# Ledicia/Molecular-Dynamics-Simulation---Lennard-Jones-monoatomic-fluid

Hardware: AMD Instinct MI355X
Metric: md_steps_per_sec_n262144_fp64 (higher is better)
Workload: dtype f64

## Files before the change

### molecular-dynamics-simulation---lennard-jones-monoatomic-fluid_amd/csrc/ljmd_kernels.hip

```cpp
#include <hip/hip_runtime.h>
#include <stdint.h>

#include "ljmd_internal.h"

namespace ljmdk {

__device__ __forceinline__ double wave_min(double v)
{
#pragma unroll
    for (int off = 32; off > 0; off >>= 1) v = fmin(v, __shfl_down(v, off, 64));
    return v;
}

__device__ __forceinline__ double wave_max(double v)
{
#pragma unroll
    for (int off = 32; off > 0; off >>= 1) v = fmax(v, __shfl_down(v, off, 64));
    return v;
}

__global__ __launch_bounds__(kBlock) void pair_rows_generic_kernel(PairArgs a)
{
    __shared__ double red[2 * kWavesPerBlock];
    const int row = blockIdx.x * kBlock + threadIdx.x;
    const double *own = a.pos + (size_t)a.rank * 3 * a.P;
    const double xi = own[row], yi = own[a.P + row], zi = own[2 * (size_t)a.P + row];

    double ax = 0.0, ay = 0.0, az = 0.0, s12 = 0.0, s6 = 0.0;

    const int j0 = blockIdx.y * a.chunk;
    const int j1 = min(j0 + a.chunk, a.n);
    for (int j = j0; j < j1;) {
        const int g = j / a.S;
        const int jl = j - g * a.S;
        const int jend = min(j1, (g + 1) * a.S);
        const double *bx = a.pos + (size_t)g * 3 * a.P;
        const double *by = bx + a.P, *bz = by + a.P;
        const int cnt = jend - j;
        const bool own_block = (g == a.rank);
        for (int k = 0; k < cnt; ++k) {
            const double dx0 = xi - bx[jl + k], dy0 = yi - by[jl + k], dz0 = zi - bz[jl + k];
            const double dx = dx0 - a.L * __builtin_round(dx0 * a.invL);
            const double dy = dy0 - a.L * __builtin_round(dy0 * a.invL);
            const double dz = dz0 - a.L * __builtin_round(dz0 * a.invL);
            const double r2 = dx * dx + dy * dy + dz * dz;
            if (r2 < a.rc2 && !(own_block && jl + k == row)) {
                const double u = 1.0 / r2;
                const double u3 = u * u * u;
                const double u6 = u3 * u3;
                s12 += u6;
                s6 += u3;
                const double mdu = 2.0 * u6 - u3;
                ax += mdu * dx * u;
                ay += mdu * dy * u;
                az += mdu * dz * u;
            }
        }
        j = jend;
    }

    double *s = a.slab + (size_t)blockIdx.y * 3 * a.P;
    s[row] = ax;
    s[a.P + row] = ay;
    s[2 * (size_t)a.P + row] = az;
    double v[2] = {s12, s6};
    block_sum<2>(v, red);
    if (threadIdx.x == 0) {
        double *w = a.wg_part + 2 * ((size_t)blockIdx.y * gridDim.x + blockIdx.x);
        w[0] = v[0];
        w[1] = v[1];
    }
}

__device__ __forceinline__ double axis_gap(double lo, double hi, double L)
{
    double g = __builtin_inf();
#pragma unroll
    for (int m = -2; m <= 2; ++m) {
        const double c = m * L;
        if (lo <= c && c <= hi) return 0.0;
        g = fmin(g, fmin(fabs(lo - c), fabs(hi - c)));
    }
    return g;
}

__device__ __forceinline__ double tile_gap2(const double *bbox, int I, int J, double L)
{
    const double *bi = bbox + (size_t)I * kBoxStride;
    const double *bj = bbox + (size_t)J * kBoxStride;
    double d2 = 0.0;
#pragma unroll
    for (int k = 0; k < 3; ++k) {
        const double g = axis_gap(bi[k] - bj[3 + k], bi[3 + k] - bj[k], L);
        d2 += g * g;
    }
    return d2;
}

__global__ __launch_bounds__(kBlock) void pair_tiles_kernel(PairArgs a)
{
    __shared__ double red[2 * kWavesPerBlock];
    const int lane = threadIdx.x & 63;
    const int wave = __builtin_amdgcn_readfirstlane(threadIdx.x >> 6);
    const int Il = blockIdx.x * kWavesPerBlock + wave;
    const int I = a.rank * a.TB + Il;
    const int row = Il * kTile + lane;
    const double *own = a.pos + (size_t)a.rank * 3 * a.P;
    const double xi = own[row], yi = own[a.P + row], zi = own[2 * (size_t)a.P + row];

    double ax = 0.0, ay = 0.0, az = 0.0, s12 = 0.0, s6 = 0.0;

    const uint64_t *mrow = a.mask + (size_t)Il * a.W;
    const int J0 = blockIdx.y * a.chunk, J1 = min(J0 + a.chunk, a.T);
    for (int w = J0 >> 6; w <= (J1 - 1) >> 6 && J0 < J1; ++w) {
        uint64_t m;
        if (a.inline_mask) {
            const int Jl = w * 64 + lane;
            const bool keep = Jl < a.T && (!(tile_gap2(a.bbox, I, Jl, a.L) > a.rc2_skin) || Jl == I);
            m = __ballot(keep);
        } else {
            m = mrow[w];
        }
        const int lo = max(J0 - w * 64, 0), hi = min(J1 - w * 64, 64);
        m &= (hi >= 64 ? ~0ull : ((1ull << hi) - 1ull)) & ~((1ull << lo) - 1ull);
        while (m) {
            const int b = __builtin_ctzll(m);
            m &= m - 1;
            const int J = w * 64 + b;
            const int gj = (a.G == 1) ? 0 : J / a.TB;
            const int jl = (J - gj * a.TB) * kTile;
            const double *bx = a.pos + (size_t)gj * 3 * a.P + jl;
            const double *by = bx + a.P, *bz = by + a.P;
            if (J == I) {
                for (int j0 = 0; j0 < kTile; j0 += 8) {
                    double xj[8], yj[8], zj[8];
#pragma unroll
                    for (int k = 0; k < 8; ++k) { xj[k] = bx[j0 + k]; yj[k] = by[j0 + k]; zj[k] = bz[j0 + k]; }
#pragma unroll
                    for (int k = 0; k < 8; ++k)
                        pair_fast<true>(xi, yi, zi, xj[k], yj[k], zj[k], a.L, a.invL, a.rc2, j0 + k == lane,
                                        ax, ay, az, s12, s6);
                }
            } else {
                for (int j0 = 0; j0 < kTile; j0 += 8) {
                    double xj[8], yj[8], zj[8];
#pragma unroll
                    for (int k = 0; k < 8; ++k) { xj[k] = bx[j0 + k]; yj[k] = by[j0 + k]; zj[k] = bz[j0 + k]; }
#pragma unroll
                    for (int k = 0; k < 8; ++k)
                        pair_fast<false>(xi, yi, zi, xj[k], yj[k], zj[k], a.L, a.invL, a.rc2, false,
                                         ax, ay, az, s12, s6);
                }
            }
        }
    }

    double *s = a.slab + (size_t)blockIdx.y * 3 * a.P;
    s[row] = ax;
    s[a.P + row] = ay;
    s[2 * (size_t)a.P + row] = az;
    double v[2] = {s12, s6};
    block_sum<2>(v, red);
    if (threadIdx.x == 0) {
        double *w = a.wg_part + 2 * ((size_t)blockIdx.y * gridDim.x + blockIdx.x);
        w[0] = v[0];
        w[1] = v[1];
    }
}


__device__ __forceinline__ double dpp_rotate(double v)
{
    int lo = __double2loint(v), hi = __double2hiint(v);
    lo = __builtin_amdgcn_update_dpp(lo, lo, 0x13C , 0xF, 0xF, false);
    hi = __builtin_amdgcn_update_dpp(hi, hi, 0x13C, 0xF, 0xF, false);
    return __hiloint2double(hi, lo);
}

__device__ __forceinline__ double straddle(double e, double half)
{
    return e - __builtin_copysign(half, e);
}

template <int NU>
__device__ __forceinline__ void pair_disp(double xi, double yi, double zi, double xj, double yj, double zj, double L,
                                          double invL, double sx, double sy, double sz, double &dx, double &dy, double &dz)
{
    static_assert(NU == 7 || NU == 8 || NU == 32 || NU == 33 || NU == 34 || NU == 40, "pair_disp: loop variant");
    dx = xi - xj; dy = yi - yj; dz = zi - zj;
    if constexpr (NU == 7) {
        dx = fma(-L, __builtin_rint(dx * invL), dx);
        dy = fma(-L, __builtin_rint(dy * invL), dy);
        dz = fma(-L, __builtin_rint(dz * invL), dz);
    }
    if constexpr (NU == 32 || NU == 40) dx = straddle(dx, sx);
    if constexpr (NU == 33 || NU == 40) dy = straddle(dy, sy);
    if constexpr (NU == 34 || NU == 40) dz = straddle(dz, sz);
}

template <bool LANE_PRED, int NU, bool INNER = false, bool ENERGY = true>
__device__ __forceinline__ void pair_n3(double xi, double yi, double zi,
                                        double xj, double yj, double zj,
                                        double L, double invL, double rc2, bool lane_ok,
                                        double sx, double sy, double sz,
                                        double &ax, double &ay, double &az,
                                        double &jx, double &jy, double &jz,
                                        double &s12, double &s6)
{
    double dx, dy, dz;
    pair_disp<NU>(xi, yi, zi, xj, yj, zj, L, invL, sx, sy, sz, dx, dy, dz);
    const double r2 = fma(dz, dz, fma(dy, dy, dx * dx));
    bool in = true;
    if constexpr (!INNER) in = r2 < rc2;
    if constexpr (LANE_PRED) in = in && lane_ok;
    if (in) {
        const double u = rcp_newton(r2);
        const double u3 = u * u * u;
        const double u6 = u3 * u3;
        if constexpr (ENERGY) {
            s12 += u6;
            s6 += u3;
        }
        const double g = fma(2.0, u6, -u3) * u;
        ax = fma(g, dx, ax);
        ay = fma(g, dy, ay);
        az = fma(g, dz, az);
        jx = fma(-g, dx, jx);
        jy = fma(-g, dy, jy);
        jz = fma(-g, dz, jz);
    }
}

template <int NU>
__device__ __forceinline__ void pair_geom(double xi, double yi, double zi, double xj, double yj, double zj, double L,
                                          double invL, double sx, double sy, double sz, double &dx, double &dy,
                                          double &dz, double &r2)
{
    pair_disp<NU>(xi, yi, zi, xj, yj, zj, L, invL, sx, sy, sz, dx, dy, dz);
    r2 = fma(dz, dz, fma(dy, dy, dx * dx));
}

template <bool INNER, bool ENERGY>
__device__ __forceinline__ void pair_apply(double u, double dx, double dy, double dz, double r2, double rc2, double &ax,
                                           double &ay, double &az, double &jx, double &jy, double &jz, double &s12,
                                           double &s6)
{
    bool in = true;
    if constexpr (!INNER) in = r2 < rc2;
    if (in) {
        const double u3 = u * u * u;
        const double u6 = u3 * u3;
        if constexpr (ENERGY) {
            s12 += u6;
            s6 += u3;
        }
        const double g = fma(2.0, u6, -u3) * u;
        ax = fma(g, dx, ax);
        ay = fma(g, dy, ay);
        az = fma(g, dz, az);
        jx = fma(-g, dx, jx);
        jy = fma(-g, dy, jy);
        jz = fma(-g, dz, jz);
    }
}

#ifndef LJMD_N3_UNROLL
#define LJMD_N3_UNROLL 8
#endif
#ifndef LJMD_BATCH_RCP
#define LJMD_BATCH_RCP 1
#endif
constexpr int kLdsAxis = 2 * kTile;

template <int RT, int NU, bool MASKED, bool INNER, bool BATCH = false, bool ENERGY = true>
__device__ __forceinline__ void column_tile_loop(const double (&xi)[RT], const double (&yi)[RT],
                                                 const double (&zi)[RT], double (&ax)[RT],
                                                 double (&ay)[RT], double (&az)[RT],
                                                 const double *park, int ns, unsigned mb,
                                                 double L, double invL, double rc2, double sx, double sy, double sz,
                                                 double &jx, double &jy, double &jz, double &s12, double &s6)
{
    static_assert(!BATCH || (!MASKED && (RT == 2 || RT == 4)), "batched reciprocal: all row tiles, 2 or 4 of them");
    static_assert(kTile / 2 % LJMD_N3_UNROLL == 0, "half a pass is a whole number of unrolled bodies");
    double xj, yj, zj;
    double nx = park[kTile], ny = park[kLdsAxis + kTile], nz = park[2 * kLdsAxis + kTile];
    for (int sb = 0; sb < ns; sb += LJMD_N3_UNROLL, park -= LJMD_N3_UNROLL) {
#pragma unroll
    for (int s = 0; s < LJMD_N3_UNROLL; ++s) {
        xj = nx; yj = ny; zj = nz;
        nx = park[kTile - 1 - s];
        ny = park[kLdsAxis + kTile - 1 - s];
        nz = park[2 * kLdsAxis + kTile - 1 - s];
        if constexpr (BATCH) {
            double dx[RT], dy[RT], dz[RT], r2[RT], u[RT];
#pragma unroll
            for (int k = 0; k < RT; ++k)
                pair_geom<NU>(xi[k], yi[k], zi[k], xj, yj, zj, L, invL, sx, sy, sz, dx[k], dy[k], dz[k], r2[k]);
            if constexpr (RT == 4) {
                const double pab = r2[0] * r2[1], pcd = r2[2] * r2[3];
                const double y = rcp_newton(pab * pcd);
                const double rab = y * pcd, rcd = y * pab;
                u[0] = r2[1] * rab; u[1] = r2[0] * rab; u[2] = r2[3] * rcd; u[3] = r2[2] * rcd;
            } else {
                const double y = rcp_newton(r2[0] * r2[1]);
                u[0] = r2[1] * y; u[1] = r2[0] * y;
            }
#pragma unroll
            for (int k = 0; k < RT; ++k)
                pair_apply<INNER, ENERGY>(u[k], dx[k], dy[k], dz[k], r2[k], rc2, ax[k], ay[k], az[k], jx, jy, jz, s12, s6);
        } else {
#pragma unroll
            for (int k = 0; k < RT; ++k)
                if (!MASKED || ((mb >> k) & 1u))
                    pair_n3<false, NU, INNER, ENERGY>(xi[k], yi[k], zi[k], xj, yj, zj, L, invL, rc2, true, sx, sy, sz,
                                              ax[k], ay[k], az[k], jx, jy, jz, s12, s6);
        }
        jx = dpp_rotate(jx); jy = dpp_rotate(jy); jz = dpp_rotate(jz);
    }
    }
}

__device__ __forceinline__ bool uniform_image(double lo, double hi, double L, double invL, double &shift)
{
    const double tlo = lo * invL, thi = hi * invL;
    const double n = __builtin_rint(0.5 * (tlo + thi));
    shift = n * L;
    return (tlo > n - 0.5 + 1e-9) && (thi < n + 0.5 - 1e-9) && (fabs(n) <= 2.0);
}

#ifdef LJMD_VARIANT_STATS
__device__ unsigned long long g_variant_stats[80];
#endif
#ifdef LJMD_WAVE_TRACE
constexpr int kTraceWaves = 1 << 16;
__device__ unsigned long long g_wave_trace[kTraceWaves * 8];
__device__ __forceinline__ unsigned long long trace_now() { return __builtin_amdgcn_s_memrealtime(); }
__device__ __forceinline__ void trace_store(unsigned wave_index, unsigned long long t0, unsigned long long t1, unsigned long long t2,
                                            unsigned heavy, unsigned item)
{
    if (wave_index >= (unsigned)kTraceWaves) return;
    const unsigned hw = __builtin_amdgcn_s_getreg((4 << 0) | (0 << 6) | (31 << 11));
    const unsigned xcc = __builtin_amdgcn_s_getreg((20 << 0) | (0 << 6) | (31 << 11));
    unsigned long long *o = g_wave_trace + (size_t)wave_index * 8;
    o[0] = t0; o[1] = t1; o[2] = t2; o[3] = trace_now(); o[4] = hw; o[5] = xcc; o[6] = heavy; o[7] = item;
}
#endif

template <int W>
__device__ __forceinline__ void wave_lds_sync()
{
    if constexpr (W == 1) {
        __syncthreads();
    } else {
        __builtin_amdgcn_fence(__ATOMIC_SEQ_CST, "wavefront");
        __builtin_amdgcn_wave_barrier();
    }
}

constexpr int kClu = 16;
constexpr int kNClu = kTile / kClu;

__device__ __forceinline__ double dpp_row_rotate(double v)
{
    int lo = __double2loint(v), hi = __double2hiint(v);
    lo = __builtin_amdgcn_update_dpp(lo, lo, 0x121 , 0xF, 0xF, false);
    hi = __builtin_amdgcn_update_dpp(hi, hi, 0x121, 0xF, 0xF, false);
    return __hiloint2double(hi, lo);
}

__device__ __forceinline__ unsigned ordered_key(float f)
{
    const unsigned b = __float_as_uint(f);
    return ((b & 0x80000000u) ? ~b : (b | 0x80000000u)) & ~63u;
}

__device__ __forceinline__ float key_value(unsigned u)
{
    u &= ~63u;
    return __uint_as_float((u & 0x80000000u) ? (u & 0x7fffffffu) : ~u);
}

template <int J>
__device__ __forceinline__ unsigned lane_xor(unsigned v)
{
    static_assert(J == 1 || J == 2 || J == 4 || J == 8 || J == 16, "lane_xor: 32 goes through v_permlane32_swap");
    if constexpr (J == 1) return (unsigned)__builtin_amdgcn_update_dpp((int)v, (int)v, 0xB1 , 0xF, 0xF, false);
    if constexpr (J == 2) return (unsigned)__builtin_amdgcn_update_dpp((int)v, (int)v, 0x4E , 0xF, 0xF, false);
    if constexpr (J == 8) return (unsigned)__builtin_amdgcn_update_dpp((int)v, (int)v, 0x128 , 0xF, 0xF, false);
    if constexpr (J == 4) return (unsigned)__builtin_amdgcn_ds_swizzle((int)v, 0x101F);
    return (unsigned)__builtin_amdgcn_ds_swizzle((int)v, 0x401F);
}

constexpr unsigned long long bitonic_min_lanes(int K, int J)
{
    unsigned long long m = 0;
    for (int l = 0; l < 64; ++l)
        if (((l & K) == 0) == ((l & J) == 0)) m |= 1ull << l;
    return m;
}

template <int K, int J>
__device__ __forceinline__ unsigned bitonic_step(unsigned key)
{
    unsigned mn, mx;
    if constexpr (J == 32) {
        const auto h = __builtin_amdgcn_permlane32_swap(key, key, false, false);
        mn = min(key, h[1]);
        mx = max(key, h[0]);
    } else {
        const unsigned other = lane_xor<J>(key);
        mn = min(key, other);
        mx = max(key, other);
    }
    constexpr unsigned long long lanes = bitonic_min_lanes(K, J);
    unsigned out;
    asm("v_cndmask_b32 %0, %1, %2, %3" : "=v"(out) : "v"(mx), "v"(mn), "s"(lanes));
    return out;
}

__device__ __forceinline__ unsigned wave_sort(unsigned key)
{
    key = bitonic_step<2, 1>(key);
    key = bitonic_step<4, 2>(key); key = bitonic_step<4, 1>(key);
    key = bitonic_step<8, 4>(key); key = bitonic_step<8, 2>(key); key = bitonic_step<8, 1>(key);
    key = bitonic_step<16, 8>(key); key = bitonic_step<16, 4>(key); key = bitonic_step<16, 2>(key);
    key = bitonic_step<16, 1>(key);
    key = bitonic_step<32, 16>(key); key = bitonic_step<32, 8>(key); key = bitonic_step<32, 4>(key);
    key = bitonic_step<32, 2>(key); key = bitonic_step<32, 1>(key);
    key = bitonic_step<64, 32>(key); key = bitonic_step<64, 16>(key); key = bitonic_step<64, 8>(key);
    key = bitonic_step<64, 4>(key); key = bitonic_step<64, 2>(key); key = bitonic_step<64, 1>(key);
    return key;
}

__device__ __forceinline__ double rows_sum(double v)
{
    unsigned lo = (unsigned)__double2loint(v), hi = (unsigned)__double2hiint(v);
    v += __hiloint2double((int)lane_xor<16>(hi), (int)lane_xor<16>(lo));
    lo = (unsigned)__double2loint(v);
    hi = (unsigned)__double2hiint(v);
    const auto l2 = __builtin_amdgcn_permlane32_swap(lo, lo, false, false);
    const auto h2 = __builtin_amdgcn_permlane32_swap(hi, hi, false, false);
    return __hiloint2double((int)h2[0], (int)l2[0]) + __hiloint2double((int)h2[1], (int)l2[1]);
}

template <int RT, bool MASKED, bool BATCH, bool ENERGY>
__device__ __forceinline__ void column_cluster_loop(const double (&xi)[RT], const double (&yi)[RT], const double (&zi)[RT],
                                                    double (&ax)[RT], double (&ay)[RT], double (&az)[RT], double xj,
                                                    double yj, double zj, const double *park, unsigned mb, double rc2,
                                                    double &jx, double &jy, double &jz, double &s12, double &s6)
{
    static_assert(!BATCH || (!MASKED && (RT == 2 || RT == 4)), "batched reciprocal: all row tiles, 2 or 4 of them");
    double nx = xj, ny = yj, nz = zj;
#pragma unroll LJMD_N3_UNROLL
    for (int s = 0; s < kClu; ++s) {
        xj = nx; yj = ny; zj = nz;
        nx = park[kClu - 1 - s];
        ny = park[kLdsAxis + kClu - 1 - s];
        nz = park[2 * kLdsAxis + kClu - 1 - s];
        if constexpr (BATCH) {
            double dx[RT], dy[RT], dz[RT], r2[RT], u[RT];
#pragma unroll
            for (int k = 0; k < RT; ++k)
                pair_geom<8>(xi[k], yi[k], zi[k], xj, yj, zj, 0.0, 0.0, 0.0, 0.0, 0.0, dx[k], dy[k], dz[k], r2[k]);
            if constexpr (RT == 4) {
                const double pab = r2[0] * r2[1], pcd = r2[2] * r2[3];
                const double y = rcp_newton(pab * pcd);
                const double rab = y * pcd, rcd = y * pab;
                u[0] = r2[1] * rab; u[1] = r2[0] * rab; u[2] = r2[3] * rcd; u[3] = r2[2] * rcd;
            } else {
                const double y = rcp_newton(r2[0] * r2[1]);
                u[0] = r2[1] * y; u[1] = r2[0] * y;
            }
#pragma unroll
            for (int k = 0; k < RT; ++k)
                pair_apply<false, ENERGY>(u[k], dx[k], dy[k], dz[k], r2[k], rc2, ax[k], ay[k], az[k], jx, jy, jz, s12, s6);
        } else {
#pragma unroll
            for (int k = 0; k < RT; ++k)
                if (!MASKED || ((mb >> k) & 1u))
                    pair_n3<false, 8, false, ENERGY>(xi[k], yi[k], zi[k], xj, yj, zj, 0.0, 0.0, rc2, true, 0.0, 0.0, 0.0,
                                                     ax[k], ay[k], az[k], jx, jy, jz, s12, s6);
        }
        jx = dpp_row_rotate(jx); jy = dpp_row_rotate(jy); jz = dpp_row_rotate(jz);
    }
}

template <int RT, bool ENERGY>
__device__ __forceinline__ void n3_cluster_pass(const N3Args &a, int lane, int Al, int c, unsigned mb, unsigned desc,
                                                const double (&xi)[RT], const double (&yi)[RT], const double (&zi)[RT],
                                                double (&ax)[RT], double (&ay)[RT], double (&az)[RT], double *parked,
                                                double *out , double &s12, double &s6)
{
    const size_t P = a.P;
    const int gj = (a.G == 1) ? 0 : c / a.TB;
    const double *cb = a.pos + (size_t)gj * 3 * P + (size_t)(c - gj * a.TB) * kTile + lane;
    double xj = cb[0], yj = cb[P], zj = cb[2 * P];
    xj += (double)((int)((desc >> 11) & 7u) - 2) * a.L;
    yj += (double)((int)((desc >> 14) & 7u) - 2) * a.L;
    zj += (double)((int)((desc >> 17) & 7u) - 2) * a.L;

    const float *d2 = a.desc2 + ((size_t)Al * a.T + c) * 8;
    const float nx = d2[0], ny = d2[1], nz = d2[2];
    float thr[4] = {d2[3], d2[4], d2[5], d2[6]};

    const float proj = (float)fma((double)nz, zj, fma((double)ny, yj, (double)nx * xj));
    const unsigned sorted = wave_sort(ordered_key(proj) | (unsigned)lane);
    const int slot = (int)(sorted & 63u);

    wave_lds_sync<1>();
    parked[lane] = xj;
    parked[kLdsAxis + lane] = yj;
    parked[2 * kLdsAxis + lane] = zj;
    wave_lds_sync<1>();
    xj = parked[slot];
    yj = parked[kLdsAxis + slot];
    zj = parked[2 * kLdsAxis + slot];
    wave_lds_sync<1>();
    const int row = lane >> 4, i = lane & (kClu - 1);
    {
        double *pk = parked + 2 * kClu * row + i;
        pk[0] = xj; pk[kClu] = xj;
        pk[kLdsAxis] = yj; pk[kLdsAxis + kClu] = yj;
        pk[2 * kLdsAxis] = zj; pk[2 * kLdsAxis + kClu] = zj;
    }
    wave_lds_sync<1>();

#pragma unroll 1
    for (int cl = 0; cl < kNClu; ++cl) {
        const float kmin = key_value((unsigned)__builtin_amdgcn_readlane((int)sorted, cl * kClu));
        unsigned mbc = 0;
#pragma unroll
        for (int k = 0; k < RT; ++k)
            if (((mb >> k) & 1u) && kmin <= thr[k]) mbc |= 1u << k;
        double jx = 0.0, jy = 0.0, jz = 0.0;
        if (mbc) {
            const double *pk = parked + 2 * kClu * cl + i;
            const double x0 = pk[kClu], y0 = pk[kLdsAxis + kClu], z0 = pk[2 * kLdsAxis + kClu];
            if (mbc == ((1u << RT) - 1u))
                column_cluster_loop<RT, false, (RT == 2 || RT == 4) && LJMD_BATCH_RCP, ENERGY>(
                    xi, yi, zi, ax, ay, az, x0, y0, z0, pk, mbc, a.rc2, jx, jy, jz, s12, s6);
            else
                column_cluster_loop<RT, true, false, ENERGY>(xi, yi, zi, ax, ay, az, x0, y0, z0, pk, mbc, a.rc2, jx, jy,
                                                             jz, s12, s6);
            jx = rows_sum(jx);
            jy = rows_sum(jy);
            jz = rows_sum(jz);
        }
#ifdef LJMD_VARIANT_STATS
        if (lane == 0) atomicAdd(&g_variant_stats[64 + __builtin_popcount(mbc)], 1ull);
#endif
        if (row == cl) {
            out[slot] = jx;
            out[kTile + slot] = jy;
            out[2 * kTile + slot] = jz;
        }
    }
}

template <int RT, int W, bool ENERGY>
__device__ __forceinline__ void n3_tile_pass(const N3Args &a, int lane, int c, int d, int l, int s0, int ns, unsigned mb,
                                             unsigned desc, const double (&xi)[RT],
                                             const double (&yi)[RT], const double (&zi)[RT], double (&ax)[RT],
                                             double (&ay)[RT], double (&az)[RT], double *parked,
                                             double &jx, double &jy, double &jz, int &s_end, double &s12, double &s6)
{
    const size_t P = a.P;
    const int gj = (a.G == 1) ? 0 : c / a.TB;
    const double *cb = a.pos + (size_t)gj * 3 * P + (size_t)(c - gj * a.TB) * kTile + lane;
    double xj = cb[0], yj = cb[P], zj = cb[2 * P];

    const int nu = (int)((desc >> 4) & 31u);
    const bool inner = ((desc >> 9) & 1u) != 0, full = ((desc >> 10) & 1u) != 0;
    const double sx = (double)((int)((desc >> 11) & 7u) - 2) * a.L;
    const double sy = (double)((int)((desc >> 14) & 7u) - 2) * a.L;
    const double sz = (double)((int)((desc >> 17) & 7u) - 2) * a.L;

    const bool diag = d == 0 && ((mb >> l) & 1u);
    const bool general_all = nu == 7 || diag;
    int loop = 7;
    double hx = 0.0, hy = 0.0, hz = 0.0;
    if (!general_all) {
        xj += sx; yj += sy; zj += sz;
        loop = 8;
        if (nu >= 27 && nu <= 30) {
            const double half = 0.5 * a.L;
            const unsigned st = (desc >> 22) & 7u, sg = (desc >> 25) & 7u;
            if (st & 1u) { hx = half; xj += (sg & 1u) ? half : -half; }
            if (st & 2u) { hy = half; yj += (sg & 2u) ? half : -half; }
            if (st & 4u) { hz = half; zj += (sg & 4u) ? half : -half; }
            loop = nu == 30 ? 40 : 32 + (nu - 27);
        }
    }
    wave_lds_sync<W>();
#pragma unroll
    for (int q = 0; q < 3; ++q) {
        const double val = q == 0 ? xj : q == 1 ? yj : zj;
        parked[q * kLdsAxis + lane] = val;
        parked[q * kLdsAxis + kTile + lane] = val;
    }
    wave_lds_sync<W>();
    if (diag) {
        const int t0 = RT == 1 ? max(s0, 1) : s0, t1 = RT == 1 ? min(s0 + ns, kTile / 2 + 1) : s0 + ns;
        const double *q0 = parked + lane + kTile;
        for (int s = t0; s < t1; ++s) {
            const double cx = q0[-s], cy = q0[kLdsAxis - s], cz = q0[2 * kLdsAxis - s];
#pragma unroll
            for (int k = 0; k < RT; ++k) {
                if (!((mb >> k) & 1u)) continue;
                if (k == l) {
                    if (s >= 1 && s <= kTile / 2)
                        pair_n3<true, 7, false, ENERGY>(xi[k], yi[k], zi[k], cx, cy, cz, a.L, a.invL, a.rc2,
                                         s < kTile / 2 || lane < kTile / 2, 0.0, 0.0, 0.0, ax[k], ay[k], az[k], jx,
                                         jy, jz, s12, s6);
                } else {
                    pair_n3<false, 7, false, ENERGY>(xi[k], yi[k], zi[k], cx, cy, cz, a.L, a.invL, a.rc2, true, 0.0,
                                      0.0, 0.0, ax[k], ay[k], az[k], jx, jy, jz, s12, s6);
                }
            }
            jx = dpp_rotate(jx); jy = dpp_rotate(jy); jz = dpp_rotate(jz);
        }
        s_end = max(t0, t1);
        return;
    }
    s_end = s0 + ns;
#define LJMD_LOOP(NU_, MASKED_, INNER_)                                                                      \
    column_tile_loop<RT, NU_, MASKED_, INNER_, false, ENERGY>(xi, yi, zi, ax, ay, az, parked + lane - s0, ns, mb, a.L, a.invL,  \
                                                  a.rc2, hx, hy, hz, jx, jy, jz, s12, s6)
#define LJMD_LOOP_ALL(NU_, INNER_)                                                                           \
    column_tile_loop<RT, NU_, false, INNER_, (RT == 2 || RT == 4) && LJMD_BATCH_RCP, ENERGY>(                              \
        xi, yi, zi, ax, ay, az, parked + lane - s0, ns, mb, a.L, a.invL, a.rc2, hx, hy, hz, jx, jy, jz, s12, s6)
    const bool all4 = mb == ((1u << RT) - 1u) && (full || !LJMD_BATCH_RCP);
#ifdef LJMD_VARIANT_STATS
    if (lane == 0)
    {
        atomicAdd(&g_variant_stats[(nu & 31) * 2 + (inner ? 1 : 0)], (unsigned long long)__builtin_popcount(mb));
        atomicAdd(&g_variant_stats[56 + __builtin_popcount(mb)], 1ull);
    }
#endif
    if (loop == 8 && inner) { if (all4) LJMD_LOOP_ALL(8, true); else LJMD_LOOP(8, true, true); }
    else if (loop == 8)     { if (all4) LJMD_LOOP_ALL(8, false); else LJMD_LOOP(8, true, false); }
    else if (loop == 32)    { if (all4) LJMD_LOOP_ALL(32, false); else LJMD_LOOP(32, true, false); }
    else if (loop == 33)    { if (all4) LJMD_LOOP_ALL(33, false); else LJMD_LOOP(33, true, false); }
    else if (loop == 34)    { if (all4) LJMD_LOOP_ALL(34, false); else LJMD_LOOP(34, true, false); }
    else if (loop == 40)    { if (all4) LJMD_LOOP_ALL(40, false); else LJMD_LOOP(40, true, false); }
    else                    { if (all4) LJMD_LOOP_ALL(7, false); else LJMD_LOOP(7, true, false); }
#undef LJMD_LOOP_ALL
#undef LJMD_LOOP
}

template <int RT>
__device__ __forceinline__ bool tile_class(const GeometryArgs &a, double invL, double rc2, int S, int Al, int c,
                                           unsigned &desc_out, unsigned *desc_far, float *desc2)
{
    {
        const int NG = a.T / RT, A = a.rank * (a.TB / RT) + Al, B = c / RT;
        int d = B - A;
        if (d < 0) d += NG;
        if (!(d == 0 || 2 * d < NG || (2 * d == NG && (A < B || a.both_ties)))) return false;
    }
    double glo[3] = {__builtin_inf(), __builtin_inf(), __builtin_inf()};
    double ghi[3] = {-__builtin_inf(), -__builtin_inf(), -__builtin_inf()};
    const double *cbx = a.bbox + (size_t)c * kBoxStride;
    unsigned mb = 0, mb_far = 0;
    bool vfar = true;
    for (int k = 0; k < RT; ++k) {
        const int tl = RT * Al + k, I = a.rank * a.TB + tl;
        const double *bb = a.bbox + (size_t)I * kBoxStride;
#pragma unroll
        for (int q = 0; q < 3; ++q) {
            glo[q] = fmin(glo[q], bb[q]);
            ghi[q] = fmax(ghi[q], bb[3 + q]);
        }
        double d2 = 0.0;
#pragma unroll
        for (int q = 0; q < 3; ++q) {
            const double g = axis_gap(bb[q] - cbx[3 + q], bb[3 + q] - cbx[q], a.L);
            d2 += g * g;
        }
        bool keep = !(d2 > a.rc2_skin) || (c == I);
        if (desc_far) {
            const bool near = (d2 <= a.rsplit2) || (c / RT == I / RT);
            mb_far |= (unsigned)(keep && !near) << k;
            if (keep && !near && !(d2 > a.rvfar2)) vfar = false;
            keep = keep && near;
        }
        mb |= (unsigned)keep << k;
    }
    if (mb == 0 && mb_far == 0) {
        desc_out = 0;
        if (desc_far) desc_far[(size_t)Al * a.T + c] = 0;
        return true;
    }
    double sx = 0.0, sy = 0.0, sz = 0.0;
    const double lo[3] = {glo[0] - cbx[3], glo[1] - cbx[4], glo[2] - cbx[5]};
    const double hi[3] = {ghi[0] - cbx[0], ghi[1] - cbx[1], ghi[2] - cbx[2]};
    const bool ux = uniform_image(lo[0], hi[0], a.L, invL, sx);
    const bool uy = uniform_image(lo[1], hi[1], a.L, invL, sy);
    const bool uz = uniform_image(lo[2], hi[2], a.L, invL, sz);
    int nu = (ux ? 0 : 1) | (uy ? 0 : 2) | (uz ? 0 : 4);
    int pq = -1;
    int pm[4] = {0, 0, 0, 0};
    if (a.pertile_images && !desc_far && RT > 1 && mb != 0 && (nu == 1 || nu == 2 || nu == 4)) {
        const int q = nu == 1 ? 0 : nu == 2 ? 1 : 2;
        int nk[4] = {0, 0, 0, 0}, nbase = 0;
        bool ok = true, have = false;
        for (int k = 0; k < RT && ok; ++k) {
            if (!((mb >> k) & 1u)) continue;
            const double *bb = a.bbox + (size_t)(a.rank * a.TB + RT * Al + k) * kBoxStride;
            double sk = 0.0;
            ok = uniform_image(bb[q] - cbx[3 + q], bb[3 + q] - cbx[q], a.L, invL, sk);
            nk[k] = (int)__builtin_rint(sk * invL);
            if (ok && !have) { nbase = nk[k]; have = true; }
            ok = ok && nk[k] - nbase >= -1 && nk[k] - nbase <= 1;
        }
        if (ok && have) {
            pq = q;
            for (int k = 0; k < RT; ++k) pm[k] = ((mb >> k) & 1u) ? nk[k] - nbase : 0;
            const double sb = (double)nbase * a.L;
            if (q == 0) sx = sb; else if (q == 1) sy = sb; else sz = sb;
            nu = 0;
        }
    }
    auto row_lo = [&](const double *bb, int k, int q) { return bb[q] - (q == pq ? (double)pm[k] * a.L : 0.0); };
    auto row_hi = [&](const double *bb, int k, int q) { return bb[3 + q] - (q == pq ? (double)pm[k] * a.L : 0.0); };
    const bool group_full = (RT * Al + RT) * kTile <= S;
    const bool full = group_full && ((c - (a.G == 1 ? 0 : c / a.TB) * a.TB) + 1) * kTile <= S;
    bool inner = nu == 0 && full && mb != 0;
    for (int k = 0; k < RT && inner; ++k) {
        if (!((mb >> k) & 1u)) continue;
        const double *bb = a.bbox + (size_t)(a.rank * a.TB + RT * Al + k) * kBoxStride;
        const double sh[3] = {sx, sy, sz};
        double far2 = 0.0;
#pragma unroll
        for (int q = 0; q < 3; ++q) {
            const double f = fmax(fabs((row_lo(bb, k, q) - cbx[3 + q]) - sh[q]), fabs((row_hi(bb, k, q) - cbx[q]) - sh[q]));
            far2 += f * f;
        }
        inner = far2 < rc2 * (1.0 - 1e-10);
    }
    unsigned straddle_axes = 0, straddle_signs = 0;
    if (nu != 0) {
        bool ok = true;
        for (int q = 0; q < 3 && ok; ++q) {
            if (!((nu >> q) & 1)) continue;
            const double tlo = lo[q] * invL, thi = hi[q] * invL;
            const double n = __builtin_rint(0.5 * (tlo + thi));
            const bool up = 0.5 * (tlo + thi) >= n;
            const double h = up ? n + 0.5 : n - 0.5;
            ok = fabs(n) <= 2.0 && tlo > h - 1.0 + 1e-9 && thi < h + 1.0 - 1e-9;
            straddle_axes |= 1u << q;
            straddle_signs |= (up ? 1u : 0u) << q;
        }
        if (ok) {
            nu = (straddle_axes == 1u) ? 27 : (straddle_axes == 2u) ? 28 : (straddle_axes == 4u) ? 29 : 30;
        } else {
            straddle_axes = straddle_signs = 0;
            sx = sy = sz = 0.0;
            nu = 7;
        }
    }
    if (nu == 0) {
        const int nz = (sx != 0.0 ? 1 : 0) | (sy != 0.0 ? 2 : 0) | (sz != 0.0 ? 4 : 0);
        nu = nz == 0 ? 8 : nz == 1 ? 16 : nz == 2 ? 17 : nz == 4 ? 18 : 0;
    }
    const int nx = (int)__builtin_rint(sx * invL), ny = (int)__builtin_rint(sy * invL), nzs = (int)__builtin_rint(sz * invL);
    unsigned cls = ((unsigned)nu << 4) | ((unsigned)inner << 9) | ((unsigned)full << 10) |
                   ((unsigned)(nx + 2) << 11) | ((unsigned)(ny + 2) << 14) | ((unsigned)(nzs + 2) << 17);
    if (pq >= 0) {
        cls |= (1u << 21) | ((unsigned)pq << 22);
        for (int k = 0; k < 4; ++k) cls |= (unsigned)(pm[k] + 1) << (24 + 2 * k);
    } else {
        cls |= (straddle_axes << 22) | (straddle_signs << 25);
    }
    if (desc2 && mb != 0 && !inner && full && c / RT != a.rank * (a.TB / RT) + Al &&
        (nu == 8 || nu == 16 || nu == 17 || nu == 18 || nu == 0)) {
        double dir[3], len2 = 0.0;
        const double sh[3] = {sx, sy, sz};
        if (pq >= 0) {
            glo[pq] = __builtin_inf();
            ghi[pq] = -__builtin_inf();
            for (int k = 0; k < RT; ++k) {
                const double *bb = a.bbox + (size_t)(a.rank * a.TB + RT * Al + k) * kBoxStride;
                glo[pq] = fmin(glo[pq], row_lo(bb, k, pq));
                ghi[pq] = fmax(ghi[pq], row_hi(bb, k, pq));
            }
        }
#pragma unroll
        for (int q = 0; q < 3; ++q) {
            dir[q] = (0.5 * (cbx[q] + cbx[3 + q]) + sh[q]) - 0.5 * (glo[q] + ghi[q]);
            len2 += dir[q] * dir[q];
        }
        if (len2 > 1.0) {
            const double inv = 1.0 / sqrt(len2);
            float nf[3];
            double nn = 0.0;
#pragma unroll
            for (int q = 0; q < 3; ++q) {
                nf[q] = (float)(dir[q] * inv);
                nn += (double)nf[q] * (double)nf[q];
            }
            if (nn <= 1.0 + 1e-6) {
                float *o = desc2 + ((size_t)Al * a.T + c) * 8;
                o[0] = nf[0]; o[1] = nf[1]; o[2] = nf[2];
                const double rc = sqrt(rc2);
                for (int k = 0; k < RT; ++k) {
                    const double *bb = a.bbox + (size_t)(a.rank * a.TB + RT * Al + k) * kBoxStride;
                    double supp = 0.0;
#pragma unroll
                    for (int q = 0; q < 3; ++q) supp += fmax((double)nf[q] * row_lo(bb, k, q), (double)nf[q] * row_hi(bb, k, q));
                    o[3 + k] = (float)(supp + rc + 1e-3);
                }
                for (int k = RT; k < 4; ++k) o[3 + k] = 0.0f;
                o[7] = 0.0f;
                double colmax = 0.0;
#pragma unroll
                for (int q = 0; q < 3; ++q) colmax += fmax((double)nf[q] * (cbx[q] + sh[q]), (double)nf[q] * (cbx[3 + q] + sh[q]));
                bool useful = false;
                for (int k = 0; k < RT; ++k) useful = useful || (((mb >> k) & 1u) && colmax > (double)o[3 + k]);
                if (useful) cls |= 1u << 20;
            }
        }
    }
    desc_out = mb | cls;
    if (desc_far) desc_far[(size_t)Al * a.T + c] = mb_far | cls | ((unsigned)(vfar && full && mb_far != 0) << 28);
    return true;
}

template <int MIN_WAVES, int RT, int W, bool ENERGY>
__global__ __launch_bounds__(kTile * W, MIN_WAVES) void pair_n3_kernel(N3Args a)
{
    __shared__ double parked_all[W][3 * kLdsAxis];
    __shared__ double comb[W > 1 ? 2 : 1][W][3][W > 1 ? kTile : 1];
    __shared__ int comb_on[2][W];
    const int lane = threadIdx.x & 63;
    const int wv = W == 1 ? 0 : __builtin_amdgcn_readfirstlane((int)(threadIdx.x >> 6));
    unsigned bx = blockIdx.x, by = blockIdx.y;
    if (a.xcd_remap) {
        const unsigned id = blockIdx.y * gridDim.x + blockIdx.x, per = gridDim.x >> 3, C = (unsigned)a.xcd_remap;
        const unsigned xcd = id & 7u, slot = id >> 3, s = slot % per;
        by = slot / per;
        bx = ((s / C) * 8u + xcd) * C + s % C;
    }
    by += (unsigned)a.by0;
#ifdef LJMD_WAVE_TRACE
    const unsigned long long tr0 = trace_now();
    unsigned long long tr1 = tr0;
    unsigned tr_heavy = 0;
#endif
    const int Al = (int)bx * W + wv;
    const bool active = Al < a.NGo;
    const int A = a.rank * a.NGo + Al;
    const int A0 = a.rank * a.NGo + (int)bx * W;
    const size_t P = a.P;
    const double *own = a.pos + (size_t)a.rank * 3 * P;

    double xi[RT], yi[RT], zi[RT];
    double ax[RT], ay[RT], az[RT];
// ... 1332 lines not shown
```

Baseline: 56.95.

## Use DPP-fused compare-exchange in wave sort and pair cross-lane reductions

Replaces the bitonic wave sort's separate shuffle, min/max and select with inline-asm DPP min/max ops, permlane16/32 swaps and row/bank-masked DPP for distance 4, driven by a constexpr sort-network table. Per-cluster readlane threshold checks become one ballot per row tile that builds a packed cluster mask before the loop. The per-cluster rows_sum reductions are replaced by pairwise permlane swap reductions across consecutive clusters, so each result is written once after four clusters. This cuts cross-lane instruction count and reduction latency, at the cost of hand-written asm with hazard-sensitive s_nop timing and a hardcoded four-cluster layout.

```diff
diff --git a/molecular-dynamics-simulation---lennard-jones-monoatomic-fluid_amd/csrc/ljmd_kernels.hip b/molecular-dynamics-simulation---lennard-jones-monoatomic-fluid_amd/csrc/ljmd_kernels.hip
--- a/molecular-dynamics-simulation---lennard-jones-monoatomic-fluid_amd/csrc/ljmd_kernels.hip
+++ b/molecular-dynamics-simulation---lennard-jones-monoatomic-fluid_amd/csrc/ljmd_kernels.hip
@@ -1,7 +1,10 @@
 #include <hip/hip_runtime.h>
 #include <stdint.h>
 
+#include <utility>
+
 #include "ljmd_internal.h"
+#include "ljmd_sortnet.h"
 
 namespace ljmdk {
 
@@ -380,67 +383,101 @@
     return __uint_as_float((u & 0x80000000u) ? (u & 0x7fffffffu) : ~u);
 }
 
-template <int J>
-__device__ __forceinline__ unsigned lane_xor(unsigned v)
-{
-    static_assert(J == 1 || J == 2 || J == 4 || J == 8 || J == 16, "lane_xor: 32 goes through v_permlane32_swap");
-    if constexpr (J == 1) return (unsigned)__builtin_amdgcn_update_dpp((int)v, (int)v, 0xB1 , 0xF, 0xF, false);
-    if constexpr (J == 2) return (unsigned)__builtin_amdgcn_update_dpp((int)v, (int)v, 0x4E , 0xF, 0xF, false);
-    if constexpr (J == 8) return (unsigned)__builtin_amdgcn_update_dpp((int)v, (int)v, 0x128 , 0xF, 0xF, false);
-    if constexpr (J == 4) return (unsigned)__builtin_amdgcn_ds_swizzle((int)v, 0x101F);
-    return (unsigned)__builtin_amdgcn_ds_swizzle((int)v, 0x401F);
-}
-
-constexpr unsigned long long bitonic_min_lanes(int K, int J)
-{
-    unsigned long long m = 0;
-    for (int l = 0; l < 64; ++l)
-        if (((l & K) == 0) == ((l & J) == 0)) m |= 1ull << l;
-    return m;
-}
-
-template <int K, int J>
+struct RowBank {
+    unsigned rows, banks;
+    bool exact;
+};
+constexpr RowBank row_bank(unsigned long long lanes, bool up)
+{
+    unsigned long long set = 0, prod = 0;
+    unsigned rows = 0, banks = 0;
+    for (int l = 0; l < kSortLanes; ++l)
+        if (((lanes >> l) & 1ull) && ((l & 4) == 0) == up) {
+            set |= 1ull << l;
+            rows |= 1u << (l >> 4);
+            banks |= 1u << ((l >> 2) & 3);
+        }
+    for (int l = 0; l < kSortLanes; ++l)
+        if (((rows >> (l >> 4)) & 1u) && ((banks >> ((l >> 2) & 3)) & 1u)) prod |= 1ull << l;
+    return {rows, banks, prod == set};
+}
+
+template <int S>
 __device__ __forceinline__ unsigned bitonic_step(unsigned key)
 {
-    unsigned mn, mx;
-    if constexpr (J == 32) {
-        const auto h = __builtin_amdgcn_permlane32_swap(key, key, false, false);
-        mn = min(key, h[1]);
-        mx = max(key, h[0]);
+    constexpr int J = kSortNet.step[S].J;
+    constexpr unsigned long long lanes = kSortNet.step[S].min_lanes;
+    constexpr unsigned lo = (unsigned)lanes, hi = (unsigned)(lanes >> 32);
+    static_assert(J == 1 || J == 2 || J == 4 || J == 8 || J == 16 || J == 32, "bitonic_step: a distance inside the wave");
+    unsigned out, mn;
+#define LJMD_CMPX_DPP(CTRL)                                                                                              \
+    asm("s_mov_b32 vcc_lo, %3\n\ts_mov_b32 vcc_hi, %4\n\t"                                                              \
+        "v_min_u32_dpp %1, %2, %2 " CTRL " row_mask:0xf bank_mask:0xf\n\t"                                              \
+        "v_max_u32_dpp %0, %2, %2 " CTRL " row_mask:0xf bank_mask:0xf\n\t"                                              \
+        "v_cndmask_b32 %0, %0, %1, vcc"                                                                                 \
+        : "=&v"(out), "=&v"(mn) : "v"(key), "i"(lo), "i"(hi) : "vcc")
+#define LJMD_CMPX_SWAP(OP)                                                                                               \
+    asm("v_mov_b32 %0, %2\n\ts_nop 1\n\t" OP " %0, %2\n\t"                                                              \
+        "s_mov_b32 vcc_lo, %3\n\ts_mov_b32 vcc_hi, %4\n\t"                                                              \
+        "v_min_u32 %1, %0, %2\n\t"                                                                                      \
+        "v_max_u32 %0, %0, %2\n\t"                                                                                      \
+        "v_cndmask_b32 %0, %0, %1, vcc"                                                                                 \
+        : "=&v"(out), "=&v"(mn), "+v"(key) : "i"(lo), "i"(hi) : "vcc")
+    if constexpr (J == 1) LJMD_CMPX_DPP("quad_perm:[1,0,3,2]");
+    else if constexpr (J == 2) LJMD_CMPX_DPP("quad_perm:[2,3,0,1]");
+    else if constexpr (J == 8) LJMD_CMPX_DPP("row_ror:8");
+    else if constexpr (J == 4) {
+        constexpr RowBank mu = row_bank(lanes, true), md = row_bank(lanes, false);
+        constexpr RowBank xu = row_bank(~lanes, true), xd = row_bank(~lanes, false);
+        static_assert(mu.exact && md.exact && xu.exact && xd.exact, "J = 4: the lane sets are rows x banks");
+        if constexpr (md.rows == 0 && xu.rows == 0)
+            asm("s_nop 1\n\t"
+                "v_min_u32_dpp %0, %1, %1 row_shl:4 row_mask:%2 bank_mask:%3\n\t"
+                "v_max_u32_dpp %0, %1, %1 row_shr:4 row_mask:%4 bank_mask:%5"
+                : "=&v"(out) : "v"(key), "i"(mu.rows), "i"(mu.banks), "i"(xd.rows), "i"(xd.banks));
+        else
+            asm("s_nop 1\n\t"
+                "v_min_u32_dpp %0, %1, %1 row_shl:4 row_mask:%2 bank_mask:%3\n\t"
+                "v_min_u32_dpp %0, %1, %1 row_shr:4 row_mask:%4 bank_mask:%5\n\t"
+                "v_max_u32_dpp %0, %1, %1 row_shl:4 row_mask:%6 bank_mask:%7\n\t"
+                "v_max_u32_dpp %0, %1, %1 row_shr:4 row_mask:%8 bank_mask:%9"
+                : "=&v"(out) : "v"(key), "i"(mu.rows), "i"(mu.banks), "i"(md.rows), "i"(md.banks), "i"(xu.rows),
+                  "i"(xu.banks), "i"(xd.rows), "i"(xd.banks));
+        (void)mn;
+    }
+    else if constexpr (J == 16) LJMD_CMPX_SWAP("v_permlane16_swap_b32");
+    else LJMD_CMPX_SWAP("v_permlane32_swap_b32");
+#undef LJMD_CMPX_DPP
+#undef LJMD_CMPX_SWAP
+    return out;
+}
+
+template <int... S>
+__device__ __forceinline__ unsigned wave_sort_steps(unsigned key, std::integer_sequence<int, S...>)
+{
+    ((key = bitonic_step<S>(key)), ...);
+    return key;
+}
+
+__device__ __forceinline__ unsigned wave_sort(unsigned key)
+{
+    return wave_sort_steps(key, std::make_integer_sequence<int, kSortSteps>());
+}
+
+template <int H>
+__device__ __forceinline__ double rows_pair(double a, double b)
+{
+    const unsigned alo = (unsigned)__double2loint(a), ahi = (unsigned)__double2hiint(a);
+    const unsigned blo = (unsigned)__double2loint(b), bhi = (unsigned)__double2hiint(b);
+    if constexpr (H == 16) {
+        const auto l = __builtin_amdgcn_permlane16_swap(alo, blo, false, false);
+        const auto h = __builtin_amdgcn_permlane16_swap(ahi, bhi, false, false);
+        return __hiloint2double((int)h[0], (int)l[0]) + __hiloint2double((int)h[1], (int)l[1]);
     } else {
-        const unsigned other = lane_xor<J>(key);
-        mn = min(key, other);
-        mx = max(key, other);
-    }
-    constexpr unsigned long long lanes = bitonic_min_lanes(K, J);
-    unsigned out;
-    asm("v_cndmask_b32 %0, %1, %2, %3" : "=v"(out) : "v"(mx), "v"(mn), "s"(lanes));
-    return out;
-}
-
-__device__ __forceinline__ unsigned wave_sort(unsigned key)
-{
-    key = bitonic_step<2, 1>(key);
-    key = bitonic_step<4, 2>(key); key = bitonic_step<4, 1>(key);
-    key = bitonic_step<8, 4>(key); key = bitonic_step<8, 2>(key); key = bitonic_step<8, 1>(key);
-    key = bitonic_step<16, 8>(key); key = bitonic_step<16, 4>(key); key = bitonic_step<16, 2>(key);
-    key = bitonic_step<16, 1>(key);
-    key = bitonic_step<32, 16>(key); key = bitonic_step<32, 8>(key); key = bitonic_step<32, 4>(key);
-    key = bitonic_step<32, 2>(key); key = bitonic_step<32, 1>(key);
-    key = bitonic_step<64, 32>(key); key = bitonic_step<64, 16>(key); key = bitonic_step<64, 8>(key);
-    key = bitonic_step<64, 4>(key); key = bitonic_step<64, 2>(key); key = bitonic_step<64, 1>(key);
-    return key;
-}
-
-__device__ __forceinline__ double rows_sum(double v)
-{
-    unsigned lo = (unsigned)__double2loint(v), hi = (unsigned)__double2hiint(v);
-    v += __hiloint2double((int)lane_xor<16>(hi), (int)lane_xor<16>(lo));
-    lo = (unsigned)__double2loint(v);
-    hi = (unsigned)__double2hiint(v);
-    const auto l2 = __builtin_amdgcn_permlane32_swap(lo, lo, false, false);
-    const auto h2 = __builtin_amdgcn_permlane32_swap(hi, hi, false, false);
-    return __hiloint2double((int)h2[0], (int)l2[0]) + __hiloint2double((int)h2[1], (int)l2[1]);
+        const auto l = __builtin_amdgcn_permlane32_swap(alo, blo, false, false);
+        const auto h = __builtin_amdgcn_permlane32_swap(ahi, bhi, false, false);
+        return __hiloint2double((int)h[0], (int)l[0]) + __hiloint2double((int)h[1], (int)l[1]);
+    }
 }
 
 template <int RT, bool MASKED, bool BATCH, bool ENERGY>
@@ -506,6 +543,16 @@
     const float proj = (float)fma((double)nz, zj, fma((double)ny, yj, (double)nx * xj));
     const unsigned sorted = wave_sort(ordered_key(proj) | (unsigned)lane);
     const int slot = (int)(sorted & 63u);
+
+    const float kmin = key_value(sorted);
+    unsigned cmask = 0;
+#pragma unroll
+    for (int k = 0; k < RT; ++k) {
+        const unsigned long long m = __builtin_amdgcn_ballot_w64(kmin <= thr[k]);
+        const unsigned lo = (unsigned)m, hi = (unsigned)(m >> 32);
+        cmask |= ((lo & 1u) | ((lo >> 12) & 0x10u) | ((hi & 1u) << 8) | ((hi >> 4) & 0x1000u)) << k;
+    }
+    cmask &= mb * 0x1111u;
 
     wave_lds_sync<1>();
     parked[lane] = xj;
@@ -525,13 +572,10 @@
     }
     wave_lds_sync<1>();
 
+    double hx = 0.0, hy = 0.0, hz = 0.0, px = 0.0, py = 0.0, pz = 0.0;
 #pragma unroll 1
     for (int cl = 0; cl < kNClu; ++cl) {
-        const float kmin = key_value((unsigned)__builtin_amdgcn_readlane((int)sorted, cl * kClu));
-        unsigned mbc = 0;
-#pragma unroll
-        for (int k = 0; k < RT; ++k)
-            if (((mb >> k) & 1u) && kmin <= thr[k]) mbc |= 1u << k;
+        const unsigned mbc = (cmask >> (4 * cl)) & 15u;
         double jx = 0.0, jy = 0.0, jz = 0.0;
         if (mbc) {
             const double *pk = parked + 2 * kClu * cl + i;
@@ -542,17 +586,21 @@
             else
                 column_cluster_loop<RT, true, false, ENERGY>(xi, yi, zi, ax, ay, az, x0, y0, z0, pk, mbc, a.rc2, jx, jy,
                                                              jz, s12, s6);
-            jx = rows_sum(jx);
-            jy = rows_sum(jy);
-            jz = rows_sum(jz);
         }
 #ifdef LJMD_VARIANT_STATS
         if (lane == 0) atomicAdd(&g_variant_stats[64 + __builtin_popcount(mbc)], 1ull);
 #endif
-        if (row == cl) {
-            out[slot] = jx;
-            out[kTile + slot] = jy;
-            out[2 * kTile + slot] = jz;
+        if ((cl & 1) == 0) {
+            hx = jx; hy = jy; hz = jz;
+        } else {
+            jx = rows_pair<16>(hx, jx); jy = rows_pair<16>(hy, jy); jz = rows_pair<16>(hz, jz);
+            if (cl == 1) {
+                px = jx; py = jy; pz = jz;
+            } else {
+                out[slot] = rows_pair<32>(px, jx);
+                out[kTile + slot] = rows_pair<32>(py, jy);
+                out[2 * kTile + slot] = rows_pair<32>(pz, jz);
+            }
         }
     }
 }
diff --git a/molecular-dynamics-simulation---lennard-jones-monoatomic-fluid_amd/csrc/ljmd_sortnet.h b/molecular-dynamics-simulation---lennard-jones-monoatomic-fluid_amd/csrc/ljmd_sortnet.h
--- /dev/null
+++ b/molecular-dynamics-simulation---lennard-jones-monoatomic-fluid_amd/csrc/ljmd_sortnet.h
@@ -0,0 +1,39 @@
+#pragma once
+
+namespace ljmdk {
+
+constexpr int kSortLanes = 64;
+constexpr int kSortSteps = 21;
+
+struct SortStep {
+    int K, J;
+    unsigned long long min_lanes;
+    unsigned char partner[kSortLanes];
+};
+
+constexpr SortStep sort_step(int K, int J)
+{
+    SortStep s{K, J, 0ull, {}};
+    for (int l = 0; l < kSortLanes; ++l) {
+        s.partner[l] = (unsigned char)(l ^ J);
+        if (((l & K) == 0) == ((l & J) == 0)) s.min_lanes |= 1ull << l;
+    }
+    return s;
+}
+
+struct SortNet {
+    SortStep step[kSortSteps];
+};
+
+constexpr SortNet make_sort_net()
+{
+    SortNet n{};
+    int k = 0;
+    for (int K = 2; K <= kSortLanes; K *= 2)
+        for (int J = K / 2; J >= 1; J /= 2) n.step[k++] = sort_step(K, J);
+    return n;
+}
+
+constexpr SortNet kSortNet = make_sort_net();
+
+}
```

New measurement: 57.52 (median of 6 runs). Within noise of the previous version (+1.0%).
